# microsoft/GenerativeImage2Text

Hardware: AMD Instinct MI355X
Metric: captions/sec whole-node (GIT_BASE 224px bs=64/GPU greedy len=20) (higher is better)
Workload: dtype f16; 1 GPU; GIT_BASE 224px bs=64/GPU greedy max_len=20 frames=1; global_batch=64, parallelism=dp1, decode_steps_per_caption=19, seq_len_returned=20, hip_graph=True, contexts_in_flight=4, layernorm_folded=True, library=libgitmi_f16.so, encoder_chains=2, schedule=mixed

## Files before the change

generativeimage2text_amd/csrc/abi_ops.hip:

```cpp
#include "../../include/gitmi.h"
#include "abi_common.h"
#include "gitmi_common.h"
#include "launchers.h"

#include <hip/hip_runtime.h>

using namespace gitmi;

#ifdef GITMI_EXPERIMENT
#include "../../include/gitmi_experiment.h"
#define GITMI_EXP_EXPORT extern "C"
#else
#define GITMI_EXP_EXPORT [[maybe_unused]] static
#endif

static inline int round_up(int x, int m) { return (x + m - 1) / m * m; }

extern "C" int gitmi_operand_dtype(void);
static const char* dtype_name(int dtype) {
    return dtype == GITMI_DTYPE_F32 ? "fp32" : dtype == GITMI_DTYPE_BF16 ? "bf16" : dtype == GITMI_DTYPE_F16 ? "fp16" : "unknown";
}
static int check_dtype(const char* op, const char* arg, int dtype) {
    if (dtype == GITMI_DTYPE_F32 || dtype == gitmi_operand_dtype()) return 0;
    return fail("%s: %s is %s (%d), but this library's 16-bit operands are %s (libgitmi%s.so)", op, arg, dtype_name(dtype), dtype,
// ... 47 lines not shown
extern "C" int gitmi_op_layernorm(const float* x, const float* gamma, const float* beta, float eps, void* y_t,
                                  float* y_f32, int rows, int D, int out_dtype, void* stream) {
    if (y_t) RCK(check_dtype("op_layernorm", "out_dtype", out_dtype));
    HIPCK(launch_layernorm(x, D, gamma, beta, eps, nullptr, y_t, D, out_dtype == GITMI_DTYPE_F32, y_f32, D, rows, D, 0, 0,
                           0, (hipStream_t)stream));
    return 0;
}
extern "C" int gitmi_op_attention(const void* qkv, void* out, int B, int N, int H, int dtype, int impl, void* stream) {
    RCK(check_dtype("op_attention", "dtype", dtype));
    const size_t esz = dtype == GITMI_DTYPE_F32 ? 4 : 2;
    const int D = H * 64;
    AttnFullArgs a{};
    a.q = qkv;
    a.k = (const char*)qkv + (size_t)D * esz;
    a.v = (const char*)qkv + (size_t)2 * D * esz;
    a.out = out;
    a.ldq = a.ldk = a.ldv = 3 * D;
    a.ldo = D;
    a.N = N; a.H = H; a.scale = 0.125f;
    if (attn_decode_configure() != hipSuccess) return fail("configure failed");
    HIPCK(launch_attn_full(a, B, dtype == GITMI_DTYPE_F32, impl, (hipStream_t)stream));
    return 0;
}

#ifdef GITMI_EXPERIMENT
static int g_dgemm_dbg = 0;
GITMI_EXP_EXPORT int gitmi_debug_set_dgemm(int dbg) { g_dgemm_dbg = dbg; return 0; }
#else
static const int g_dgemm_dbg = 0;
#endif
extern "C" int gitmi_op_dgemm(const void* A, const void* W, const float* bias, const float* colsum, const float* stats,
                              int strips, float eps, void* C, int c_frag, int M, int N, int K, int act, int strips_per_wg,
                              void* stream) {
    DGemmArgs g{};
    g.dbg = g_dgemm_dbg;
    g.strips_per_wg = strips_per_wg;
    g.c_frag = c_frag;
    if (c_frag && N % 32) return fail("op_dgemm: a fragment-major output needs N %% 32 == 0");
    g.A = (const unsigned short*)A; g.lda = K; g.W = (const unsigned short*)W; g.bias = bias;
    if (stats) { g.colsum = colsum; g.stats_in = (const float2*)stats; g.strips_in = strips; g.inv_d = 1.0f / (float)K; g.eps_in = eps; }
    g.C = C; g.ldc = N; g.act = act; g.M = M; g.N = N; g.K = K;
    if (K % 32) return fail("op_dgemm: K must be a multiple of 32");
    HIPCK(launch_dgemm(g, (hipStream_t)stream));
    return 0;
}
extern "C" int gitmi_op_dgemm_res(const void* A, const void* W, const float* bias, const float* res_x, const float* res_stats,
// ... 302 lines not shown
```

generativeimage2text_amd/csrc/kernels_attn.hip:

```cpp
#include "gitmi_common.h"
#include "launchers.h"
#include <type_traits>

namespace gitmi {

constexpr int HD = 64;

template <typename T>
__global__ __launch_bounds__(256) void attn_full_valu_kernel(AttnFullArgs a) {
    __shared__ float Ks[64][HD + 1];
    __shared__ float Vs[64][HD + 1];
    __shared__ float qs[16][HD];
    __shared__ float ps[16][64];

    const int tid = threadIdx.x, lane = tid & 63, wave = tid >> 6;
    const int h = blockIdx.y, b = blockIdx.z;
    const int q0 = blockIdx.x * 16;
    const T* Q = reinterpret_cast<const T*>(a.q);
    const T* K = reinterpret_cast<const T*>(a.k);
    const T* V = reinterpret_cast<const T*>(a.v);
    T* O = reinterpret_cast<T*>(a.out);
    const size_t base_row = (size_t)b * a.N;
    const int n = a.ntok ? a.ntok[b] : a.N;
    if (q0 >= n) {
// ... 179 lines not shown
                    o_acc[t][dt] = mfma16(vf.v, pf, o_acc[t][dt]);
                }
            }
        }
    }

#pragma unroll
    for (int t = 0; t < QT; ++t) {
        const int qr = qbase + (t * 4 + wave) * 16 + l15;
        if (qr < a.N) {
            const float inv = qr < n ? 1.0f / l_run[t] : 0.f;
            bf16_t* op = O + (base_row + qr) * a.ldo + h * HD;
#pragma unroll
            for (int dt = 0; dt < 4; ++dt) {
                uint2 tt;
                tt.x = pack2bf(o_acc[t][dt][0] * inv, o_acc[t][dt][1] * inv);
                tt.y = pack2bf(o_acc[t][dt][2] * inv, o_acc[t][dt][3] * inv);
                *reinterpret_cast<uint2*>(op + dt * 16 + lg * 4) = tt;
            }
        }
    }
}

template <int NSUB, bool RAGGED = false>
__global__ __launch_bounds__(256, 2) void attn_full_mfma_short_kernel(AttnFullArgs a) {
    constexpr int NK = NSUB * 16;
    constexpr int NB = (NSUB + 1) / 2;
    constexpr int LDV = NB * 32 + 8;
    static_assert((LDV / 8) % 2 == 1, "V^T row stride must be an odd multiple of 16 bytes");
    __shared__ __attribute__((aligned(16))) bf16_t Ks[NK * FA_LDK];
    __shared__ __attribute__((aligned(16))) bf16_t Vt[HD * LDV];

    const int tid = threadIdx.x, lane = tid & 63, wave = tid >> 6;
    const int l15 = lane & 15, lg = lane >> 4;
    const int h = blockIdx.x, b = blockIdx.y;
    const bf16_t* Q = reinterpret_cast<const bf16_t*>(a.q);
    const bf16_t* K = reinterpret_cast<const bf16_t*>(a.k);
    const bf16_t* V = reinterpret_cast<const bf16_t*>(a.v);
    bf16_t* O = reinterpret_cast<bf16_t*>(a.out);
    const size_t base_row = (size_t)b * a.N;
    const int n = RAGGED ? a.ntok[b] : a.N;
    if constexpr (RAGGED) {
        for (int i = tid; i < (a.N - n) * 8; i += 256) {
            const int qr = n + (i >> 3);
            *reinterpret_cast<u32x4_t*>(O + (base_row + qr) * a.ldo + h * HD + (i & 7) * 8) = u32x4_t{0u, 0u, 0u, 0u};
        }
    }

#pragma unroll
    for (int it = 0; it < (NK * 8 + 255) / 256; ++it) {
        int idx = tid + it * 256;
        const bool ok = idx < NK * 8;
        idx = ok ? idx : NK * 8 - 1;
        const int key = idx >> 3, c = idx & 7;
        const int kr = key < n ? key : n - 1;
        const u32x4_t kc = *reinterpret_cast<const u32x4_t*>(K + (base_row + kr) * a.ldk + h * HD + c * 8);
        if (ok) *reinterpret_cast<u32x4_t*>(Ks + key * FA_LDK + c * 8) = kc;
    }
#pragma unroll
    for (int it = 0; it < (NB * 8 * 8 + 255) / 256; ++it) {
        int task = tid + it * 256;
        const bool ok = task < NB * 8 * 8;
        task = ok ? task : NB * 8 * 8 - 1;
        const int kg = task % (NB * 8), c = task / (NB * 8);
        u32x4_t vc[4];
#pragma unroll
        for (int e = 0; e < 4; ++e) {
            const int key = kg * 4 + e;
            const int kr = key < n ? key : n - 1;
            vc[e] = *reinterpret_cast<const u32x4_t*>(V + (base_row + kr) * a.ldv + h * HD + c * 8);
            if (key >= n) vc[e] = u32x4_t{0u, 0u, 0u, 0u};
        }
        if (ok) {
#pragma unroll
            for (int w = 0; w < 4; ++w) {
                uint2 even, odd;
                even.x = (vc[0][w] & 0xffffu) | (vc[1][w] << 16);
                even.y = (vc[2][w] & 0xffffu) | (vc[3][w] << 16);
                odd.x = (vc[0][w] >> 16) | (vc[1][w] & 0xffff0000u);
                odd.y = (vc[2][w] >> 16) | (vc[3][w] & 0xffff0000u);
                *reinterpret_cast<uint2*>(Vt + (c * 8 + 2 * w) * LDV + kg * 4) = even;
                *reinterpret_cast<uint2*>(Vt + (c * 8 + 2 * w + 1) * LDV + kg * 4) = odd;
            }
        }
    }
    __syncthreads();

    const int nqt = (n + 15) >> 4;
    const float c2 = a.scale * 1.4426950408889634f;

    auto process = [&](auto nt_c, int t0) {
        constexpr int NT = decltype(nt_c)::value;
        bf16x8_t qf[NT][2];
#pragma unroll
        for (int u = 0; u < NT; ++u) {
            int qr = (t0 + 4 * u) * 16 + l15;
            qr = qr < n ? qr : n - 1;
            const bf16_t* qp = Q + (base_row + qr) * a.ldq + h * HD + lg * 8;
            qf[u][0] = *reinterpret_cast<const bf16x8_t*>(qp);
            qf[u][1] = *reinterpret_cast<const bf16x8_t*>(qp + 32);
        }
        f32x4_t sacc[NT][NSUB];
#pragma unroll
        for (int st_ = 0; st_ < NSUB; ++st_) {
            const bf16x8_t kf0 = *reinterpret_cast<const bf16x8_t*>(Ks + (st_ * 16 + l15) * FA_LDK + lg * 8);
            const bf16x8_t kf1 = *reinterpret_cast<const bf16x8_t*>(Ks + (st_ * 16 + l15) * FA_LDK + 32 + lg * 8);
#pragma unroll
            for (int u = 0; u < NT; ++u) {
                sacc[u][st_] = mfma16(kf0, qf[u][0], f32x4_t{0.f, 0.f, 0.f, 0.f});
                sacc[u][st_] = mfma16(kf1, qf[u][1], sacc[u][st_]);
            }
            if constexpr (NSUB > 13) { if (st_ % 4 == 3) __builtin_amdgcn_sched_barrier(0); }
        }
        float inv_l[NT];
#pragma unroll
        for (int u = 0; u < NT; ++u) {
            if constexpr (RAGGED) {
#pragma unroll
                for (int st_ = 0; st_ < NSUB; ++st_)
#pragma unroll
                    for (int r = 0; r < 4; ++r)
                        if (st_ * 16 + lg * 4 + r >= n) sacc[u][st_][r] = -INFINITY;
            } else {
#pragma unroll
                for (int r = 0; r < 4; ++r)
                    if ((NSUB - 1) * 16 + lg * 4 + r >= a.N) sacc[u][NSUB - 1][r] = -INFINITY;
            }
            float m = -INFINITY;
#pragma unroll
            for (int st_ = 0; st_ < NSUB; ++st_)
#pragma unroll
                for (int r = 0; r < 4; ++r) m = fmaxf(m, sacc[u][st_][r]);
            m = fmaxf(m, __shfl_xor(m, 16, 64));
            m = fmaxf(m, __shfl_xor(m, 32, 64));
            const float mc = m * c2;
            float psum = 0.f;
#pragma unroll
            for (int st_ = 0; st_ < NSUB; ++st_)
#pragma unroll
                for (int r = 0; r < 4; ++r) {
                    const float p = __builtin_amdgcn_exp2f(sacc[u][st_][r] * c2 - mc);
                    sacc[u][st_][r] = p;
                    psum += p;
                }
            psum += __shfl_xor(psum, 16, 64);
            psum += __shfl_xor(psum, 32, 64);
            inv_l[u] = 1.0f / psum;
        }
        uint32_t pk2[NT][NSUB][2];
#pragma unroll
        for (int u = 0; u < NT; ++u)
#pragma unroll
            for (int st_ = 0; st_ < NSUB; ++st_) {
                pk2[u][st_][0] = pack2bf(sacc[u][st_][0], sacc[u][st_][1]);
                pk2[u][st_][1] = pack2bf(sacc[u][st_][2], sacc[u][st_][3]);
            }
        f32x4_t o_acc[NT][4];
#pragma unroll
        for (int u = 0; u < NT; ++u)
#pragma unroll
            for (int dt = 0; dt < 4; ++dt) o_acc[u][dt] = f32x4_t{0.f, 0.f, 0.f, 0.f};
#pragma unroll
        for (int blk = 0; blk < NB; ++blk) {
            bf16x8_t pf[NT];
#pragma unroll
            for (int u = 0; u < NT; ++u) {
                union { bf16x8_t v; uint32_t w[4]; } pk;
                pk.w[0] = pk2[u][2 * blk][0];
                pk.w[1] = pk2[u][2 * blk][1];
                const bool has1 = 2 * blk + 1 < NSUB;
                const int s1 = has1 ? 2 * blk + 1 : 0;
                pk.w[2] = has1 ? pk2[u][s1][0] : 0u;
                pk.w[3] = has1 ? pk2[u][s1][1] : 0u;
                pf[u] = pk.v;
            }
#pragma unroll
            for (int dt = 0; dt < 4; ++dt) {
                union { bf16x8_t v; uint2 h2[2]; } vf;
                const bf16_t* vp = Vt + (dt * 16 + l15) * LDV + blk * 32 + lg * 4;
                vf.h2[0] = *reinterpret_cast<const uint2*>(vp);
                vf.h2[1] = *reinterpret_cast<const uint2*>(vp + 16);
#pragma unroll
                for (int u = 0; u < NT; ++u)
                    o_acc[u][dt] = mfma16(vf.v, pf[u], o_acc[u][dt]);
            }
        }
#pragma unroll
        for (int u = 0; u < NT; ++u) {
            const int qr = (t0 + 4 * u) * 16 + l15;
            if (qr < n) {
                bf16_t* op = O + (base_row + qr) * a.ldo + h * HD;
#pragma unroll
                for (int dt = 0; dt < 4; ++dt) {
                    uint2 tt;
                    tt.x = pack2bf(o_acc[u][dt][0] * inv_l[u], o_acc[u][dt][1] * inv_l[u]);
                    tt.y = pack2bf(o_acc[u][dt][2] * inv_l[u], o_acc[u][dt][3] * inv_l[u]);
                    *reinterpret_cast<uint2*>(op + dt * 16 + lg * 4) = tt;
                }
            }
        }
    };

    for (int t0 = wave; t0 < nqt; t0 += 8) {
        if (t0 + 4 < nqt) process(std::integral_constant<int, 2>{}, t0);
        else process(std::integral_constant<int, 1>{}, t0);
    }
}

template <typename T>
__global__ void kv_repack_kernel(const T* __restrict__ qkv, T* __restrict__ kh, T* __restrict__ vh, int B, int N, int H,
                                 int d) {
    constexpr int CH = 16 / (int)sizeof(T);
    constexpr int CPH = HD / CH;
    const size_t per = (size_t)B * H * N * CPH;
    for (size_t i = blockIdx.x * (size_t)blockDim.x + threadIdx.x; i < 2 * per; i += (size_t)gridDim.x * blockDim.x) {
        const int kv = i >= per;
        size_t r = kv ? i - per : i;
        const int c = (int)(r % CPH); r /= CPH;
        const int n = (int)(r % N); r /= N;
        const int h = (int)(r % H);
        const int b = (int)(r / H);
        const T* src = qkv + ((size_t)b * N + n) * 3 * d + (kv ? 2 : 1) * d + h * HD + c * CH;
        T* dst = (kv ? vh : kh) + (((size_t)b * H + h) * N + n) * HD + c * CH;
        *reinterpret_cast<u32x4_t*>(dst) = *reinterpret_cast<const u32x4_t*>(src);
    }
}

template <typename T> struct Raw8;
// ... 231 lines not shown
        }
    }
    __syncthreads();
    for (int i = tid; i < k * HD; i += 256) {
        const int j = i / HD, dd = i % HD;
        float mm = -INFINITY;
#pragma unroll
        for (int w = 0; w < 4; ++w) mm = fmaxf(mm, part[w][j][HD]);
        float num = 0.f, den = 0.f;
#pragma unroll
        for (int w = 0; w < 4; ++w) {
            const float mw = part[w][j][HD];
            const float aw = mw == -INFINITY ? 0.f : fast_exp(mw - mm);
            num += aw * part[w][j][dd];
            den += aw * part[w][j][HD + 1];
        }
        if constexpr (sizeof(T) == 2) {
            if (a.out_frag) { O[frag_offset(row0 + j, h * HD + dd, a.d >> 5)] = f2bf(num / den); continue; }
        }
        st<T>(O + (size_t)(row0 + j) * a.d + h * HD + dd, num / den);
    }
}

hipError_t launch_attn_full(const AttnFullArgs& a, int B, bool is_f32, int impl, hipStream_t s) {
    if (B <= 0 || a.N <= 0) return hipSuccess;
    if (impl == 1) {
        if (is_f32) return hipErrorInvalidValue;
        const int nsub = (a.N + 15) / 16;
        if (nsub == 13 && a.ntok) hipLaunchKernelGGL((attn_full_mfma_short_kernel<13, true>), dim3(a.H, B), dim3(256), 0, s, a);
        else if (nsub == 13) hipLaunchKernelGGL(attn_full_mfma_short_kernel<13>, dim3(a.H, B), dim3(256), 0, s, a);
        else if (nsub == 17 && a.ntok) hipLaunchKernelGGL((attn_full_mfma_short_kernel<17, true>), dim3(a.H, B), dim3(256), 0, s, a);
        else if (nsub == 17) hipLaunchKernelGGL(attn_full_mfma_short_kernel<17>, dim3(a.H, B), dim3(256), 0, s, a);
        else hipLaunchKernelGGL(attn_full_mfma_kernel, dim3((a.N + 255) / 256, a.H, B), dim3(256), 0, s, a);
    } else if (impl == 2) {
        if (is_f32) return hipErrorInvalidValue;
        hipLaunchKernelGGL(attn_full_mfma_kernel, dim3((a.N + 255) / 256, a.H, B), dim3(256), 0, s, a);
    } else if (is_f32) {
        hipLaunchKernelGGL(attn_full_valu_kernel<float>, dim3((a.N + 15) / 16, a.H, B), dim3(256), 0, s, a);
    } else {
        hipLaunchKernelGGL(attn_full_valu_kernel<bf16_t>, dim3((a.N + 15) / 16, a.H, B), dim3(256), 0, s, a);
    }
    return hipGetLastError();
}

hipError_t launch_kv_repack(const void* qkv, void* kh, void* vh, int B, int N, int H, int d, bool is_f32, hipStream_t s) {
    if (B <= 0 || N <= 0) return hipSuccess;
    const size_t total = 2 * (size_t)B * H * N * (is_f32 ? 16 : 8);
    size_t grid = (total + 255) / 256;
    grid = grid > 8192 ? 8192 : grid;
    if (is_f32) hipLaunchKernelGGL(kv_repack_kernel<float>, dim3((int)grid), dim3(256), 0, s, (const float*)qkv, (float*)kh,
                                   (float*)vh, B, N, H, d);
    else hipLaunchKernelGGL(kv_repack_kernel<bf16_t>, dim3((int)grid), dim3(256), 0, s, (const bf16_t*)qkv, (bf16_t*)kh,
                            (bf16_t*)vh, B, N, H, d);
    return hipGetLastError();
}

hipError_t attn_decode_configure() { return hipSuccess; }

size_t attn_decode_lds_bytes(int beams, int N_img, int pos) {
// ... 22 lines not shown
```

generativeimage2text_amd/csrc/launchers.h:

```cpp
#pragma once
#include <hip/hip_runtime.h>
#include <stddef.h>

namespace gitmi {

struct GemmArgs {
    const void* A; const void* W; const float* bias; const float* res; void* C;
    int M, N, K;
    int lda, ldc, ldr;
    int act;
    int tiles_n, nwg;
    int ng;
    int dbg;
    int out_f16;
    int shared;
    const float2* ln_part; int ln_nparts; const float* ln_colsum; float ln_inv_d, ln_eps;
    float2* part_out;
    const float2* res_part; int res_nparts; const float* res_gamma; const float* res_beta; float res_inv_d, res_eps;
};
bool gemm_uses_p8(const GemmArgs& g, bool in_f32, bool out_f32);
hipError_t launch_gemm(const GemmArgs& g, bool in_f32, bool out_f32, hipStream_t s);
hipError_t launch_gemm_p8(GemmArgs g, bool out_f32, hipStream_t s);
bool gemm_p8_supports(const GemmArgs& g);
int gemm_p8_cost(const GemmArgs& g, int bm);
// ... 54 lines not shown
                                  int nparts, hipStream_t s);
hipError_t launch_layernorm_s16(const void* x, int ldx, const float* gamma, const float* beta, float eps,
                                const float* add_after, void* y_t, int ld_t, bool t_is_f32, void* y_s, int ld_s,
                                int rows, int D, int map_n_in, int map_n_out, int map_off, hipStream_t s);
hipError_t launch_embed_ln(const int* ids, int ld_ids, int pos, const float* words, const float* positions,
                           const float* gamma, const float* beta, float eps, float* h_f, void* h_t, bool t_is_f32,
                           int R, int D, int vocab, bool frag, hipStream_t s);
hipError_t launch_frag_pack(const void* src_bf16, void* dst_bf16, int rows, int rows_out, int K, hipStream_t s);
hipError_t launch_convert_pad(const float* src, void* dst, bool dst_f32, size_t rows, int K, int Kpad,
                              hipStream_t s);
hipError_t launch_convert(const void* src, bool src_f32, void* dst, bool dst_f32, size_t n, hipStream_t s);
hipError_t launch_chain_input(const float* x, void* xb_frag, float2* stats, int R, int d, hipStream_t s);
hipError_t launch_copy_f32(const float* src, int lds, float* dst, int ldd, int rows, int cols, hipStream_t s);
hipError_t launch_fill_i32(int* dst, int value, int n, hipStream_t s);

struct AttnFullArgs {
    const void* q; const void* k; const void* v; void* out;
    int ldq, ldk, ldv, ldo;
    int N, H;
    float scale;
    const int* ntok;
};
hipError_t launch_attn_full(const AttnFullArgs& a, int B, bool is_f32, int impl, hipStream_t s);

struct AttnDecodeArgs {
    const void* qkv; const void* img_k; const void* img_v; void* txt_k; void* txt_v; void* out;
    const int* kv_src;
    const int* img_of;
    int ld_src;
    int d;
    int N_img, T_max, pos, beams;
    int N_pad;
    int out_frag;
    float scale;
    int dbg;
    int pairs_per_wg;
    int pairs_per_wave;
    int stream_wgs;
    int n_pairs;
    int waves_per_pair;
    const int* ntok;
};
hipError_t launch_kv_repack(const void* qkv, void* kh, void* vh, int B, int N, int H, int d, bool is_f32, hipStream_t s);
size_t attn_decode_lds_bytes(int beams, int N_img, int pos);
hipError_t launch_attn_decode(const AttnDecodeArgs& a, int B, int H, bool is_f32, hipStream_t s);
hipError_t launch_kv_repack_frag(const void* qkv, void* kf, void* vt, int B, int N, int N_pad, int H, int d, hipStream_t s);
// ... 92 lines not shown
```

generativeimage2text_amd/engine.py:

```python
from __future__ import annotations

import ctypes as C
import os
from typing import Dict, List, Mapping, Optional, Sequence, Tuple

import torch

_HERE = os.path.dirname(os.path.abspath(__file__))
LIB_PATH = os.path.join(_HERE, "libgitmi.so")
LIB_PATH_F16 = os.path.join(_HERE, "libgitmi_f16.so")
LIB_PATH_EXP = os.path.join(_HERE, "libgitmi_exp.so")

PREC_BF16, PREC_F32 = 0, 1
DTYPE_F32, DTYPE_BF16, DTYPE_F16 = 0, 1, 2
DTYPE_F16_STREAM = 3
SEARCH_AUTOREGRESSIVE, SEARCH_GENERATOR, SEARCH_TRIE = 0, 1, 2
SEARCH_SCORE = 3
SEARCH_ATTEND = 4
ACT_NONE, ACT_QUICKGELU, ACT_GELU_ERF = 0, 1, 2

EXPORTED_SYMBOLS = [
    "gitmi_abi_version", "gitmi_last_error", "gitmi_create", "gitmi_destroy", "gitmi_load_tensor",
    "gitmi_finalize_weights", "gitmi_encode_frames", "gitmi_prefill", "gitmi_step_logits",
    "gitmi_generate", "gitmi_search_begin", "gitmi_search_rows", "gitmi_search_advance",
    "gitmi_search_finish", "gitmi_profile_enable", "gitmi_profile_read", "gitmi_set_graph",
    "gitmi_op_gemm", "gitmi_op_layernorm", "gitmi_op_attention", "gitmi_op_dgemm", "gitmi_op_dgemm_res",
    "gitmi_op_vocab_topm", "gitmi_clone", "gitmi_op_attn_decode", "gitmi_preprocess_image",
    "gitmi_set_image_shape", "gitmi_preprocess_image_to", "gitmi_generate_prefixed", "gitmi_set_temporal_embedding", "gitmi_op_kv_repack", "gitmi_set_encode_after", "gitmi_op_sample_rows",
    "gitmi_search_done_count", "gitmi_set_trie", "gitmi_operand_dtype", "gitmi_set_shared_device", "gitmi_preprocess_batch",
    "gitmi_set_ln_fold", "gitmi_op_gemm_ln",
]
EXPERIMENT_SYMBOLS = [
    "gitmi_debug_import_stage", "gitmi_debug_head_from", "gitmi_debug_set_gemm_impl", "gitmi_debug_set_dgemm",
    "gitmi_debug_score_attn", "gitmi_debug_score_head", "gitmi_debug_attention_ragged", "gitmi_debug_attn_decode_ragged",
    "gitmi_debug_vocab_topm_rules", "gitmi_debug_search_begin_prefixed", "gitmi_debug_search_advance_lists", "gitmi_debug_read_hidden",
    "gitmi_debug_im2col", "gitmi_debug_pos_resize", "gitmi_debug_vit_assemble", "gitmi_debug_ragged_front", "gitmi_debug_zero_pad_rows",
    "gitmi_debug_layernorm_map", "gitmi_debug_score_attn_map",
]


class GitmiConfig(C.Structure):
    _fields_ = [(n, C.c_int32) for n in (
        "image_size", "patch", "vit_width", "vit_layers", "vit_heads", "dec_hidden", "dec_layers",
        "dec_heads", "dec_ffn", "vocab", "max_pos", "num_frames", "sos", "eos", "precision",
        "max_batch", "max_beams", "max_frames", "max_text_len", "max_image_pixels", "max_image_tokens")]


class GitmiSearch(C.Structure):
    _fields_ = [("kind", C.c_int32), ("beam_size", C.c_int32), ("per_node_beam_size", C.c_int32),
                ("max_steps", C.c_int32), ("length_penalty", C.c_double),
                ("do_sample", C.c_int32), ("top_k", C.c_int32), ("top_p", C.c_double), ("temperature", C.c_double),
                ("seed", C.c_uint64), ("repetition_penalty", C.c_double),
                ("num_keep_best", C.c_int32), ("reserved_", C.c_int32)]


class GitmiProfile(C.Structure):
    _fields_ = [("vit_ms", C.c_float), ("prefill_ms", C.c_float), ("decode_ms", C.c_float),
                ("total_ms", C.c_float), ("gemm_ms", C.c_float), ("gemm_launches", C.c_int32),
                ("gemm_flops", C.c_double), ("vit_gemm_ms", C.c_float), ("vit_gemm_launches", C.c_int32),
                ("vit_gemm_flops", C.c_double), ("decode_step_ms", C.c_float), ("decode_steps", C.c_int32),
# ... 803 lines not shown
    _ck(_experiment_only(lib, "gitmi_debug_vocab_topm_rules")(
        *ops, eps, *shape, _ptr(ids), 0 if ids is None else int(ids.shape[1]), int(cur_len), _ptr(plen), int(beams),
        int(suppress_kind), float(rep_penalty), *outs, int(max_wgs), _stream()), lib)
    return result


def set_gemm_impl(impl: int) -> None:
    lib = load_library()
    _ck(_experiment_only(lib, "gitmi_debug_set_gemm_impl")(int(impl)), lib)


def op_attn_decode(qkv, img_k, img_v, txt_k, txt_v, kv_src, B, H, N_img, T_max, pos, beams, dbg=0):
    lib = _op_library(qkv.dtype, img_k.dtype, img_v.dtype, txt_k.dtype, txt_v.dtype, fp32_ok=True)
    R, d = B * beams, H * 64
    out = torch.empty(R, d, device=qkv.device, dtype=qkv.dtype)
    if qkv.dtype != torch.float32 and img_k.dim() == 4:
        img_k, img_v = kv_repack(img_k, img_v)
    _ck(lib.gitmi_op_attn_decode(qkv.data_ptr(), img_k.data_ptr(), img_v.data_ptr(), txt_k.data_ptr(), txt_v.data_ptr(),
                                 kv_src.data_ptr(), out.data_ptr(), B, H, N_img, T_max, pos, beams, _torch_dtype_code(qkv),
                                 dbg, _stream()), lib)
    return out


def op_attention_ragged(qkv: torch.Tensor, ntok, B: int, N: int, H: int, impl: int) -> torch.Tensor:
    lib = load_library()
    nt = torch.as_tensor(ntok, dtype=torch.int32).to(qkv.device)
    out = torch.empty(B * N, H * 64, device=qkv.device, dtype=qkv.dtype)
    _ck(_experiment_only(lib, "gitmi_debug_attention_ragged")(qkv.data_ptr(), out.data_ptr(), nt.data_ptr(), B, N, H,
                                                              _torch_dtype_code(qkv), impl, _stream()), lib)
    return out


def op_attn_decode_ragged(qkv, img_k, img_v, txt_k, txt_v, kv_src, ntok, B, H, N_img, T_max, pos, beams):
    lib = load_library()
    R, d = B * beams, H * 64
    nt = torch.as_tensor(ntok, dtype=torch.int32).to(qkv.device)
    out = torch.empty(R, d, device=qkv.device, dtype=qkv.dtype)
    if qkv.dtype != torch.float32 and img_k.dim() == 4:
        img_k, img_v = kv_repack(img_k, img_v)
    _ck(_experiment_only(lib, "gitmi_debug_attn_decode_ragged")(qkv.data_ptr(), img_k.data_ptr(), img_v.data_ptr(), txt_k.data_ptr(),
                                                                txt_v.data_ptr(), kv_src.data_ptr(), out.data_ptr(), nt.data_ptr(), B,
                                                                H, N_img, T_max, pos, beams, _torch_dtype_code(qkv), _stream()), lib)
    return out


def op_score_attn(qkv: torch.Tensor, img_kv: torch.Tensor, image_of: torch.Tensor, Q: int, H: int, N_img: int,
# ... 144 lines not shown
```

include/gitmi_experiment.h:

```cpp
#ifndef GITMI_EXPERIMENT_H_
#define GITMI_EXPERIMENT_H_
#include "gitmi.h"
#ifdef __cplusplus
extern "C" {
#endif

int  gitmi_debug_import_stage(gitmi_engine* dst, gitmi_engine* src, int stage, void* stream);
int  gitmi_debug_head_from(gitmi_engine* dst, gitmi_engine* src, int R, float* logits_out, void* stream);

int  gitmi_debug_set_gemm_impl(int impl);

int  gitmi_debug_set_dgemm(int dbg);

int  gitmi_debug_score_attn(const void* qkv, const void* img_kv, const int* image_of, void* out, int Q, int H, int N_img, int Lp,
                            int dtype, void* stream);
int  gitmi_debug_score_attn_map(const void* qkv, const void* img_kv, const int* image_of, const int* ntok, float* out, int Q, int H,
                                int N_img, int Lp, int dtype, void* stream);
int  gitmi_debug_score_head(const void* A, const void* W, const float* bias, const int* tgt, int M, int V, int K, int dtype,
                            float* out, void* stream);

int  gitmi_debug_attention_ragged(const void* qkv, void* out, const int* ntok, int B, int N, int H, int dtype, int impl, void* stream);
int  gitmi_debug_attn_decode_ragged(const void* qkv, const void* img_k, const void* img_v, void* txt_k, void* txt_v,
                                    const int* kv_src, void* out, const int* ntok, int B, int H, int N_img, int T_max, int pos,
                                    int beams, int dtype, void* stream);

int  gitmi_debug_vocab_topm_rules(const void* A, const void* W, const float* bias, const float* colsum, const float* stats,
                                  int strips, float eps, int M, int V, int K, int cols_per_wg, int mtop, const int* ids, int ld_ids,
                                  int cur_len, const int* plen, int beams, int suppress_kind, float rep_penalty, float* part_val,
                                  int* part_idx, float* part_lse, float* logits_out, int max_wgs, void* stream);
int  gitmi_debug_search_begin_prefixed(gitmi_engine* e, const gitmi_search* sp, int B, const int64_t* start_host, int ld,
                                       const int32_t* plen_host, int vocab, void* stream);
int  gitmi_debug_search_advance_lists(gitmi_engine* e, const float* part_val, const int* part_idx, const float* part_lse,
                                      int nparts, int slots, int embed, void* stream);
int  gitmi_debug_read_hidden(gitmi_engine* e, int R, float* hf_out, void* ht_out, int* ht_frag, int* ht_dtype, void* stream);

// ... 18 lines not shown
```

Measured before the change: 11620 captions/s.

## Add persistent double-buffered short attention kernel overlapping next head's K/V load

For the non-ragged short-sequence encoder attention (13 or 17 key subtiles), impl 1 now launches a persistent 512-thread kernel with one workgroup per CU. Each workgroup loops over (batch, head) pairs and prefetches the next pair's K/V into registers while computing the current one, then writes them into a second LDS buffer. The tile math is factored into shared helpers, and the old per-pair kernel moves to experimental impl 3. The aim is to hide global-load latency and cut workgroup launch overhead. The cost is doubled LDS, more register pressure and one workgroup per CU, which can limit occupancy.

```diff
diff --git a/generativeimage2text_amd/csrc/abi_ops.hip b/generativeimage2text_amd/csrc/abi_ops.hip
--- a/generativeimage2text_amd/csrc/abi_ops.hip
+++ b/generativeimage2text_amd/csrc/abi_ops.hip
@@ -93,6 +93,8 @@
     HIPCK(launch_attn_full(a, B, dtype == GITMI_DTYPE_F32, impl, (hipStream_t)stream));
     return 0;
 }
+
+GITMI_EXP_EXPORT int gitmi_debug_attn_short_grid(int pairs) { return attn_full_short_grid(pairs); }
 
 #ifdef GITMI_EXPERIMENT
 static int g_dgemm_dbg = 0;
diff --git a/generativeimage2text_amd/csrc/kernels_attn.hip b/generativeimage2text_amd/csrc/kernels_attn.hip
--- a/generativeimage2text_amd/csrc/kernels_attn.hip
+++ b/generativeimage2text_amd/csrc/kernels_attn.hip
@@ -225,188 +225,310 @@
     }
 }
 
+template <int NSUB> struct ShortGeom {
+    static constexpr int NK = NSUB * 16;
+    static constexpr int NB = (NSUB + 1) / 2;
+    static constexpr int LDV = NB * 32 + 8;
+    static_assert((LDV / 8) % 2 == 1, "V^T row stride must be an odd multiple of 16 bytes");
+    static constexpr int KS = NK * FA_LDK;
+    static constexpr int VT = HD * LDV;
+};
+
+struct ShortPair {
+    int h, n;
+    size_t base_row;
+};
+template <bool RAGGED> __device__ __forceinline__ ShortPair short_pair(const AttnFullArgs& a, int b, int h) {
+    ShortPair p;
+    p.h = h;
+    p.n = RAGGED ? a.ntok[b] : a.N;
+    p.base_row = (size_t)b * a.N;
+    return p;
+}
+
+template <int NSUB, int NTHR> struct ShortStage {
+    using G = ShortGeom<NSUB>;
+    static constexpr int KCH = G::NK * 8, VTASK = G::NB * 8 * 8;
+    static constexpr int KIT = KCH / NTHR, KREM = KCH - KIT * NTHR;
+    static constexpr int VIT = VTASK / NTHR, VREM = VTASK - VIT * NTHR;
+    static_assert(VREM % 64 == 0 && KREM % 4 == 0 && VREM + KREM / 4 <= NTHR, "the shared last block does not fit");
+    u32x4_t kc[KIT];
+    u32x4_t vc[VIT + 1][4];
+
+    static __device__ __forceinline__ u32x4_t chunk(const bf16_t* M, int ld, const ShortPair& p, int key, int c) {
+        const int kr = key < p.n ? key : p.n - 1;
+        return *reinterpret_cast<const u32x4_t*>(M + (p.base_row + kr) * ld + p.h * HD + c * 8);
+    }
+    __device__ __forceinline__ void load(const AttnFullArgs& a, const ShortPair& p, int tid) {
+        const bf16_t* K = reinterpret_cast<const bf16_t*>(a.k);
+        const bf16_t* V = reinterpret_cast<const bf16_t*>(a.v);
+#pragma unroll
+        for (int it = 0; it < KIT; ++it) {
+            const int idx = tid + it * NTHR;
+            kc[it] = chunk(K, a.ldk, p, idx >> 3, idx & 7);
+        }
+#pragma unroll
+        for (int it = 0; it <= VIT; ++it) {
+            const int task = tid + it * NTHR;
+            if (it < VIT || tid < VREM) {
+                const int kg = task % (G::NB * 8), c = task / (G::NB * 8);
+#pragma unroll
+                for (int e = 0; e < 4; ++e) vc[it][e] = chunk(V, a.ldv, p, kg * 4 + e, c);
+            } else if (tid - VREM < KREM / 4) {
+                const int idx = KIT * NTHR + (tid - VREM) * 4;
+#pragma unroll
+                for (int e = 0; e < 4; ++e) vc[it][e] = chunk(K, a.ldk, p, idx >> 3, (idx & 7) + e);
+            }
+        }
+    }
+    __device__ __forceinline__ void store(bf16_t* Ks, bf16_t* Vt, int tid, int n) const {
+#pragma unroll
+        for (int it = 0; it < KIT; ++it) {
+            const int idx = tid + it * NTHR;
+            *reinterpret_cast<u32x4_t*>(Ks + (idx >> 3) * FA_LDK + (idx & 7) * 8) = kc[it];
+        }
+#pragma unroll
+        for (int it = 0; it <= VIT; ++it) {
+            const int task = tid + it * NTHR;
+            if (it < VIT || tid < VREM) {
+                const int kg = task % (G::NB * 8), c = task / (G::NB * 8);
+                u32x4_t v[4];
+#pragma unroll
+                for (int e = 0; e < 4; ++e) v[e] = kg * 4 + e < n ? vc[it][e] : u32x4_t{0u, 0u, 0u, 0u};
+#pragma unroll
+                for (int w = 0; w < 4; ++w) {
+                    uint2 even, odd;
+                    even.x = (v[0][w] & 0xffffu) | (v[1][w] << 16);
+                    even.y = (v[2][w] & 0xffffu) | (v[3][w] << 16);
+                    odd.x = (v[0][w] >> 16) | (v[1][w] & 0xffff0000u);
+                    odd.y = (v[2][w] >> 16) | (v[3][w] & 0xffff0000u);
+                    *reinterpret_cast<uint2*>(Vt + (c * 8 + 2 * w) * G::LDV + kg * 4) = even;
+                    *reinterpret_cast<uint2*>(Vt + (c * 8 + 2 * w + 1) * G::LDV + kg * 4) = odd;
+                }
+            } else if (tid - VREM < KREM / 4) {
+                const int idx = KIT * NTHR + (tid - VREM) * 4;
+#pragma unroll
+                for (int e = 0; e < 4; ++e)
+                    *reinterpret_cast<u32x4_t*>(Ks + (idx >> 3) * FA_LDK + ((idx & 7) + e) * 8) = vc[it][e];
+            }
+        }
+    }
+};
+
+template <int NT>
+__device__ __forceinline__ void short_load_q(const AttnFullArgs& a, const ShortPair& p, int t0, int ts, int l15, int lg,
+                                             bf16x8_t (&qf)[NT][2]) {
+    const bf16_t* Q = reinterpret_cast<const bf16_t*>(a.q);
+#pragma unroll
+    for (int u = 0; u < NT; ++u) {
+        int qr = (t0 + ts * u) * 16 + l15;
+        qr = qr < p.n ? qr : p.n - 1;
+        const bf16_t* qp = Q + (p.base_row + qr) * a.ldq + p.h * HD + lg * 8;
+        qf[u][0] = *reinterpret_cast<const bf16x8_t*>(qp);
+        qf[u][1] = *reinterpret_cast<const bf16x8_t*>(qp + 32);
+    }
+}
+
+template <int NSUB, bool RAGGED, int NT, int QS>
+__device__ __forceinline__ void short_tile_math(const AttnFullArgs& a, const ShortPair& p, const bf16_t* Ks, const bf16_t* Vt,
+                                                const bf16x8_t (&qf)[QS][2], int t0, int ts, int l15, int lg) {
+    using G = ShortGeom<NSUB>;
+    constexpr int NB = G::NB, LDV = G::LDV;
+    bf16_t* O = reinterpret_cast<bf16_t*>(a.out);
+    const int n = p.n;
+    const float c2 = a.scale * 1.4426950408889634f;
+    f32x4_t sacc[NT][NSUB];
+#pragma unroll
+    for (int st_ = 0; st_ < NSUB; ++st_) {
+        const bf16x8_t kf0 = *reinterpret_cast<const bf16x8_t*>(Ks + (st_ * 16 + l15) * FA_LDK + lg * 8);
+        const bf16x8_t kf1 = *reinterpret_cast<const bf16x8_t*>(Ks + (st_ * 16 + l15) * FA_LDK + 32 + lg * 8);
+#pragma unroll
+        for (int u = 0; u < NT; ++u) {
+            sacc[u][st_] = mfma16(kf0, qf[u][0], f32x4_t{0.f, 0.f, 0.f, 0.f});
+            sacc[u][st_] = mfma16(kf1, qf[u][1], sacc[u][st_]);
+        }
+        if constexpr (NSUB > 13) { if (st_ % 4 == 3) __builtin_amdgcn_sched_barrier(0); }
+    }
+    float inv_l[NT];
+#pragma unroll
+    for (int u = 0; u < NT; ++u) {
+        if constexpr (RAGGED) {
+#pragma unroll
+            for (int st_ = 0; st_ < NSUB; ++st_)
+#pragma unroll
+                for (int r = 0; r < 4; ++r)
+                    if (st_ * 16 + lg * 4 + r >= n) sacc[u][st_][r] = -INFINITY;
+        } else {
+#pragma unroll
+            for (int r = 0; r < 4; ++r)
+                if ((NSUB - 1) * 16 + lg * 4 + r >= a.N) sacc[u][NSUB - 1][r] = -INFINITY;
+        }
+        float m = -INFINITY;
+#pragma unroll
+        for (int st_ = 0; st_ < NSUB; ++st_)
+#pragma unroll
+            for (int r = 0; r < 4; ++r) m = fmaxf(m, sacc[u][st_][r]);
+        m = fmaxf(m, __shfl_xor(m, 16, 64));
+        m = fmaxf(m, __shfl_xor(m, 32, 64));
+        const float mc = m * c2;
+        float psum = 0.f;
+#pragma unroll
+        for (int st_ = 0; st_ < NSUB; ++st_)
+#pragma unroll
+            for (int r = 0; r < 4; ++r) {
+                const float pr = __builtin_amdgcn_exp2f(sacc[u][st_][r] * c2 - mc);
+                sacc[u][st_][r] = pr;
+                psum += pr;
+            }
+        psum += __shfl_xor(psum, 16, 64);
+        psum += __shfl_xor(psum, 32, 64);
+        inv_l[u] = 1.0f / psum;
+    }
+    uint32_t pk2[NT][NSUB][2];
+#pragma unroll
+    for (int u = 0; u < NT; ++u)
+#pragma unroll
+        for (int st_ = 0; st_ < NSUB; ++st_) {
+            pk2[u][st_][0] = pack2bf(sacc[u][st_][0], sacc[u][st_][1]);
+            pk2[u][st_][1] = pack2bf(sacc[u][st_][2], sacc[u][st_][3]);
+        }
+    f32x4_t o_acc[NT][4];
+#pragma unroll
+    for (int u = 0; u < NT; ++u)
+#pragma unroll
+        for (int dt = 0; dt < 4; ++dt) o_acc[u][dt] = f32x4_t{0.f, 0.f, 0.f, 0.f};
+#pragma unroll
+    for (int blk = 0; blk < NB; ++blk) {
+        bf16x8_t pf[NT];
+#pragma unroll
+        for (int u = 0; u < NT; ++u) {
+            union { bf16x8_t v; uint32_t w[4]; } pk;
+            pk.w[0] = pk2[u][2 * blk][0];
+            pk.w[1] = pk2[u][2 * blk][1];
+            const bool has1 = 2 * blk + 1 < NSUB;
+            const int s1 = has1 ? 2 * blk + 1 : 0;
+            pk.w[2] = has1 ? pk2[u][s1][0] : 0u;
+            pk.w[3] = has1 ? pk2[u][s1][1] : 0u;
+            pf[u] = pk.v;
+        }
+#pragma unroll
+        for (int dt = 0; dt < 4; ++dt) {
+            union { bf16x8_t v; uint2 h2[2]; } vf;
+            const bf16_t* vp = Vt + (dt * 16 + l15) * LDV + blk * 32 + lg * 4;
+            vf.h2[0] = *reinterpret_cast<const uint2*>(vp);
+            vf.h2[1] = *reinterpret_cast<const uint2*>(vp + 16);
+#pragma unroll
+            for (int u = 0; u < NT; ++u)
+                o_acc[u][dt] = mfma16(vf.v, pf[u], o_acc[u][dt]);
+        }
+    }
+#pragma unroll
+    for (int u = 0; u < NT; ++u) {
+        const int qr = (t0 + ts * u) * 16 + l15;
+        if (qr < n) {
+            bf16_t* op = O + (p.base_row + qr) * a.ldo + p.h * HD;
+#pragma unroll
+            for (int dt = 0; dt < 4; ++dt) {
+                uint2 tt;
+                tt.x = pack2bf(o_acc[u][dt][0] * inv_l[u], o_acc[u][dt][1] * inv_l[u]);
+                tt.y = pack2bf(o_acc[u][dt][2] * inv_l[u], o_acc[u][dt][3] * inv_l[u]);
+                *reinterpret_cast<uint2*>(op + dt * 16 + lg * 4) = tt;
+            }
+        }
+    }
+}
+
+template <int NTHR> __device__ __forceinline__ void short_zero_pad(const AttnFullArgs& a, const ShortPair& p, int tid) {
+    bf16_t* O = reinterpret_cast<bf16_t*>(a.out);
+    for (int i = tid; i < (a.N - p.n) * 8; i += NTHR) {
+        const int qr = p.n + (i >> 3);
+        *reinterpret_cast<u32x4_t*>(O + (p.base_row + qr) * a.ldo + p.h * HD + (i & 7) * 8) = u32x4_t{0u, 0u, 0u, 0u};
+    }
+}
+
+#define SHORT_LDS_BARRIER()                                \
+    do {                                                   \
+        asm volatile("s_waitcnt lgkmcnt(0)" ::: "memory"); \
+        __builtin_amdgcn_s_barrier();                      \
+    } while (0)
+
+template <int NSUB>
+__global__ __launch_bounds__(512) void attn_full_mfma_short_persistent_kernel(AttnFullArgs a, int pairs) {
+    using G = ShortGeom<NSUB>;
+    constexpr bool RAGGED = false;
+    constexpr int TS = 8;
+    constexpr int NTM = NSUB <= 13 ? 2 : 1;
+    __shared__ __attribute__((aligned(16))) bf16_t Ks[2 * G::KS];
+    __shared__ __attribute__((aligned(16))) bf16_t Vt[2 * G::VT];
+
+    const int tid = threadIdx.x, lane = tid & 63, wave = tid >> 6;
+    const int l15 = lane & 15, lg = lane >> 4;
+    const int grid = gridDim.x;
+
+    int pair = blockIdx.x;
+    ShortPair p = short_pair<RAGGED>(a, pair / a.H, pair % a.H);
+    ShortStage<NSUB, 512> stg;
+    bf16x8_t qf[NTM][2];
+    stg.load(a, p, tid);
+    short_load_q<NTM>(a, p, wave, TS, l15, lg, qf);
+    stg.store(Ks, Vt, tid, p.n);
+    SHORT_LDS_BARRIER();
+
+    int cur = 0;
+    for (;;) {
+        const int next = pair + grid;
+        const bool has_next = next < pairs;
+        ShortPair pn = p;
+        if (has_next) {
+            pn = short_pair<RAGGED>(a, next / a.H, next % a.H);
+            stg.load(a, pn, tid);
+        }
+        __builtin_amdgcn_sched_barrier(0);
+
+        const bf16_t* ks = Ks + cur * G::KS;
+        const bf16_t* vt = Vt + cur * G::VT;
+        const int nqt = (p.n + 15) >> 4;
+        if (NTM == 2 && wave + TS < nqt) short_tile_math<NSUB, RAGGED, NTM>(a, p, ks, vt, qf, wave, TS, l15, lg);
+        else if (wave < nqt) short_tile_math<NSUB, RAGGED, 1>(a, p, ks, vt, qf, wave, TS, l15, lg);
+        for (int t0 = wave + NTM * TS; t0 < nqt; t0 += NTM * TS) {
+            bf16x8_t qx[NTM][2];
+            short_load_q<NTM>(a, p, t0, TS, l15, lg, qx);
+            if (NTM == 2 && t0 + TS < nqt) short_tile_math<NSUB, RAGGED, NTM>(a, p, ks, vt, qx, t0, TS, l15, lg);
+            else short_tile_math<NSUB, RAGGED, 1>(a, p, ks, vt, qx, t0, TS, l15, lg);
+        }
+        if (!has_next) break;
+
+        __builtin_amdgcn_sched_barrier(0);
+        stg.store(Ks + (cur ^ 1) * G::KS, Vt + (cur ^ 1) * G::VT, tid, pn.n);
+        short_load_q<NTM>(a, pn, wave, TS, l15, lg, qf);
+        SHORT_LDS_BARRIER();
+        pair = next;
+        p = pn;
+        cur ^= 1;
+    }
+}
+
 template <int NSUB, bool RAGGED = false>
 __global__ __launch_bounds__(256, 2) void attn_full_mfma_short_kernel(AttnFullArgs a) {
-    constexpr int NK = NSUB * 16;
-    constexpr int NB = (NSUB + 1) / 2;
-    constexpr int LDV = NB * 32 + 8;
-    static_assert((LDV / 8) % 2 == 1, "V^T row stride must be an odd multiple of 16 bytes");
-    __shared__ __attribute__((aligned(16))) bf16_t Ks[NK * FA_LDK];
-    __shared__ __attribute__((aligned(16))) bf16_t Vt[HD * LDV];
+    using G = ShortGeom<NSUB>;
+    __shared__ __attribute__((aligned(16))) bf16_t Ks[G::KS];
+    __shared__ __attribute__((aligned(16))) bf16_t Vt[G::VT];
 
     const int tid = threadIdx.x, lane = tid & 63, wave = tid >> 6;
     const int l15 = lane & 15, lg = lane >> 4;
-    const int h = blockIdx.x, b = blockIdx.y;
-    const bf16_t* Q = reinterpret_cast<const bf16_t*>(a.q);
-    const bf16_t* K = reinterpret_cast<const bf16_t*>(a.k);
-    const bf16_t* V = reinterpret_cast<const bf16_t*>(a.v);
-    bf16_t* O = reinterpret_cast<bf16_t*>(a.out);
-    const size_t base_row = (size_t)b * a.N;
-    const int n = RAGGED ? a.ntok[b] : a.N;
-    if constexpr (RAGGED) {
-        for (int i = tid; i < (a.N - n) * 8; i += 256) {
-            const int qr = n + (i >> 3);
-            *reinterpret_cast<u32x4_t*>(O + (base_row + qr) * a.ldo + h * HD + (i & 7) * 8) = u32x4_t{0u, 0u, 0u, 0u};
-        }
-    }
-
-#pragma unroll
-    for (int it = 0; it < (NK * 8 + 255) / 256; ++it) {
-        int idx = tid + it * 256;
-        const bool ok = idx < NK * 8;
-        idx = ok ? idx : NK * 8 - 1;
-        const int key = idx >> 3, c = idx & 7;
-        const int kr = key < n ? key : n - 1;
-        const u32x4_t kc = *reinterpret_cast<const u32x4_t*>(K + (base_row + kr) * a.ldk + h * HD + c * 8);
-        if (ok) *reinterpret_cast<u32x4_t*>(Ks + key * FA_LDK + c * 8) = kc;
-    }
-#pragma unroll
-    for (int it = 0; it < (NB * 8 * 8 + 255) / 256; ++it) {
-        int task = tid + it * 256;
-        const bool ok = task < NB * 8 * 8;
-        task = ok ? task : NB * 8 * 8 - 1;
-        const int kg = task % (NB * 8), c = task / (NB * 8);
-        u32x4_t vc[4];
-#pragma unroll
-        for (int e = 0; e < 4; ++e) {
-            const int key = kg * 4 + e;
-            const int kr = key < n ? key : n - 1;
-            vc[e] = *reinterpret_cast<const u32x4_t*>(V + (base_row + kr) * a.ldv + h * HD + c * 8);
-            if (key >= n) vc[e] = u32x4_t{0u, 0u, 0u, 0u};
-        }
-        if (ok) {
-#pragma unroll
-            for (int w = 0; w < 4; ++w) {
-                uint2 even, odd;
-                even.x = (vc[0][w] & 0xffffu) | (vc[1][w] << 16);
-                even.y = (vc[2][w] & 0xffffu) | (vc[3][w] << 16);
-                odd.x = (vc[0][w] >> 16) | (vc[1][w] & 0xffff0000u);
-                odd.y = (vc[2][w] >> 16) | (vc[3][w] & 0xffff0000u);
-                *reinterpret_cast<uint2*>(Vt + (c * 8 + 2 * w) * LDV + kg * 4) = even;
-                *reinterpret_cast<uint2*>(Vt + (c * 8 + 2 * w + 1) * LDV + kg * 4) = odd;
-            }
-        }
-    }
+    const ShortPair p = short_pair<RAGGED>(a, blockIdx.y, blockIdx.x);
+    if constexpr (RAGGED) short_zero_pad<256>(a, p, tid);
+    ShortStage<NSUB, 256> stg;
+    stg.load(a, p, tid);
+    stg.store(Ks, Vt, tid, p.n);
     __syncthreads();
 
-    const int nqt = (n + 15) >> 4;
-    const float c2 = a.scale * 1.4426950408889634f;
-
-    auto process = [&](auto nt_c, int t0) {
-        constexpr int NT = decltype(nt_c)::value;
-        bf16x8_t qf[NT][2];
-#pragma unroll
-        for (int u = 0; u < NT; ++u) {
-            int qr = (t0 + 4 * u) * 16 + l15;
-            qr = qr < n ? qr : n - 1;
-            const bf16_t* qp = Q + (base_row + qr) * a.ldq + h * HD + lg * 8;
-            qf[u][0] = *reinterpret_cast<const bf16x8_t*>(qp);
-            qf[u][1] = *reinterpret_cast<const bf16x8_t*>(qp + 32);
-        }
-        f32x4_t sacc[NT][NSUB];
-#pragma unroll
-        for (int st_ = 0; st_ < NSUB; ++st_) {
-            const bf16x8_t kf0 = *reinterpret_cast<const bf16x8_t*>(Ks + (st_ * 16 + l15) * FA_LDK + lg * 8);
-            const bf16x8_t kf1 = *reinterpret_cast<const bf16x8_t*>(Ks + (st_ * 16 + l15) * FA_LDK + 32 + lg * 8);
-#pragma unroll
-            for (int u = 0; u < NT; ++u) {
-                sacc[u][st_] = mfma16(kf0, qf[u][0], f32x4_t{0.f, 0.f, 0.f, 0.f});
-                sacc[u][st_] = mfma16(kf1, qf[u][1], sacc[u][st_]);
-            }
-            if constexpr (NSUB > 13) { if (st_ % 4 == 3) __builtin_amdgcn_sched_barrier(0); }
-        }
-        float inv_l[NT];
-#pragma unroll
-        for (int u = 0; u < NT; ++u) {
-            if constexpr (RAGGED) {
-#pragma unroll
-                for (int st_ = 0; st_ < NSUB; ++st_)
-#pragma unroll
-                    for (int r = 0; r < 4; ++r)
-                        if (st_ * 16 + lg * 4 + r >= n) sacc[u][st_][r] = -INFINITY;
-            } else {
-#pragma unroll
-                for (int r = 0; r < 4; ++r)
-                    if ((NSUB - 1) * 16 + lg * 4 + r >= a.N) sacc[u][NSUB - 1][r] = -INFINITY;
-            }
-            float m = -INFINITY;
-#pragma unroll
-            for (int st_ = 0; st_ < NSUB; ++st_)
-#pragma unroll
-                for (int r = 0; r < 4; ++r) m = fmaxf(m, sacc[u][st_][r]);
-            m = fmaxf(m, __shfl_xor(m, 16, 64));
-            m = fmaxf(m, __shfl_xor(m, 32, 64));
-            const float mc = m * c2;
-            float psum = 0.f;
-#pragma unroll
-            for (int st_ = 0; st_ < NSUB; ++st_)
-#pragma unroll
-                for (int r = 0; r < 4; ++r) {
-                    const float p = __builtin_amdgcn_exp2f(sacc[u][st_][r] * c2 - mc);
-                    sacc[u][st_][r] = p;
-                    psum += p;
-                }
-            psum += __shfl_xor(psum, 16, 64);
-            psum += __shfl_xor(psum, 32, 64);
-            inv_l[u] = 1.0f / psum;
-        }
-        uint32_t pk2[NT][NSUB][2];
-#pragma unroll
-        for (int u = 0; u < NT; ++u)
-#pragma unroll
-            for (int st_ = 0; st_ < NSUB; ++st_) {
-                pk2[u][st_][0] = pack2bf(sacc[u][st_][0], sacc[u][st_][1]);
-                pk2[u][st_][1] = pack2bf(sacc[u][st_][2], sacc[u][st_][3]);
-            }
-        f32x4_t o_acc[NT][4];
-#pragma unroll
-        for (int u = 0; u < NT; ++u)
-#pragma unroll
-            for (int dt = 0; dt < 4; ++dt) o_acc[u][dt] = f32x4_t{0.f, 0.f, 0.f, 0.f};
-#pragma unroll
-        for (int blk = 0; blk < NB; ++blk) {
-            bf16x8_t pf[NT];
-#pragma unroll
-            for (int u = 0; u < NT; ++u) {
-                union { bf16x8_t v; uint32_t w[4]; } pk;
-                pk.w[0] = pk2[u][2 * blk][0];
-                pk.w[1] = pk2[u][2 * blk][1];
-                const bool has1 = 2 * blk + 1 < NSUB;
-                const int s1 = has1 ? 2 * blk + 1 : 0;
-                pk.w[2] = has1 ? pk2[u][s1][0] : 0u;
-                pk.w[3] = has1 ? pk2[u][s1][1] : 0u;
-                pf[u] = pk.v;
-            }
-#pragma unroll
-            for (int dt = 0; dt < 4; ++dt) {
-                union { bf16x8_t v; uint2 h2[2]; } vf;
-                const bf16_t* vp = Vt + (dt * 16 + l15) * LDV + blk * 32 + lg * 4;
-                vf.h2[0] = *reinterpret_cast<const uint2*>(vp);
-                vf.h2[1] = *reinterpret_cast<const uint2*>(vp + 16);
-#pragma unroll
-                for (int u = 0; u < NT; ++u)
-                    o_acc[u][dt] = mfma16(vf.v, pf[u], o_acc[u][dt]);
-            }
-        }
-#pragma unroll
-        for (int u = 0; u < NT; ++u) {
-            const int qr = (t0 + 4 * u) * 16 + l15;
-            if (qr < n) {
-                bf16_t* op = O + (base_row + qr) * a.ldo + h * HD;
-#pragma unroll
-                for (int dt = 0; dt < 4; ++dt) {
-                    uint2 tt;
-                    tt.x = pack2bf(o_acc[u][dt][0] * inv_l[u], o_acc[u][dt][1] * inv_l[u]);
-                    tt.y = pack2bf(o_acc[u][dt][2] * inv_l[u], o_acc[u][dt][3] * inv_l[u]);
-                    *reinterpret_cast<uint2*>(op + dt * 16 + lg * 4) = tt;
-                }
-            }
-        }
-    };
-
+    const int nqt = (p.n + 15) >> 4;
     for (int t0 = wave; t0 < nqt; t0 += 8) {
-        if (t0 + 4 < nqt) process(std::integral_constant<int, 2>{}, t0);
-        else process(std::integral_constant<int, 1>{}, t0);
+        bf16x8_t qf[2][2];
+        short_load_q<2>(a, p, t0, 4, l15, lg, qf);
+        if (t0 + 4 < nqt) short_tile_math<NSUB, RAGGED, 2>(a, p, Ks, Vt, qf, t0, 4, l15, lg);
+        else short_tile_math<NSUB, RAGGED, 1>(a, p, Ks, Vt, qf, t0, 4, l15, lg);
     }
 }
 
@@ -684,9 +806,42 @@
     }
 }
 
+int attn_full_short_grid(int pairs) {
+    static int cus[64];
+    int dev = 0;
+    if (hipGetDevice(&dev) != hipSuccess || dev < 0 || dev >= 64) return 0;
+    int n = __atomic_load_n(&cus[dev], __ATOMIC_RELAXED);
+    if (n <= 0) {
+        if (hipDeviceGetAttribute(&n, hipDeviceAttributeMultiprocessorCount, dev) != hipSuccess || n <= 0) return 0;
+        __atomic_store_n(&cus[dev], n, __ATOMIC_RELAXED);
+    }
+    return pairs < n ? pairs : n;
+}
+
+template <int NSUB>
+static hipError_t launch_short_persistent(const AttnFullArgs& a, int B, hipStream_t s) {
+    const int pairs = B * a.H;
+    const int grid = attn_full_short_grid(pairs);
+    if (grid <= 0) return hipErrorInvalidDevice;
+    hipLaunchKernelGGL(attn_full_mfma_short_persistent_kernel<NSUB>, dim3(grid), dim3(512), 0, s, a, pairs);
+    return hipGetLastError();
+}
+
 hipError_t launch_attn_full(const AttnFullArgs& a, int B, bool is_f32, int impl, hipStream_t s) {
     if (B <= 0 || a.N <= 0) return hipSuccess;
     if (impl == 1) {
+        if (is_f32) return hipErrorInvalidValue;
+        const int nsub = (a.N + 15) / 16;
+        if (nsub == 13 && a.ntok) hipLaunchKernelGGL((attn_full_mfma_short_kernel<13, true>), dim3(a.H, B), dim3(256), 0, s, a);
+        else if (nsub == 13) return launch_short_persistent<13>(a, B, s);
+        else if (nsub == 17 && a.ntok) hipLaunchKernelGGL((attn_full_mfma_short_kernel<17, true>), dim3(a.H, B), dim3(256), 0, s, a);
+        else if (nsub == 17) return launch_short_persistent<17>(a, B, s);
+        else hipLaunchKernelGGL(attn_full_mfma_kernel, dim3((a.N + 255) / 256, a.H, B), dim3(256), 0, s, a);
+    } else if (impl == 2) {
+        if (is_f32) return hipErrorInvalidValue;
+        hipLaunchKernelGGL(attn_full_mfma_kernel, dim3((a.N + 255) / 256, a.H, B), dim3(256), 0, s, a);
+    } else if (impl == 3) {
+#ifdef GITMI_EXPERIMENT
         if (is_f32) return hipErrorInvalidValue;
         const int nsub = (a.N + 15) / 16;
         if (nsub == 13 && a.ntok) hipLaunchKernelGGL((attn_full_mfma_short_kernel<13, true>), dim3(a.H, B), dim3(256), 0, s, a);
@@ -694,9 +849,9 @@
         else if (nsub == 17 && a.ntok) hipLaunchKernelGGL((attn_full_mfma_short_kernel<17, true>), dim3(a.H, B), dim3(256), 0, s, a);
         else if (nsub == 17) hipLaunchKernelGGL(attn_full_mfma_short_kernel<17>, dim3(a.H, B), dim3(256), 0, s, a);
         else hipLaunchKernelGGL(attn_full_mfma_kernel, dim3((a.N + 255) / 256, a.H, B), dim3(256), 0, s, a);
-    } else if (impl == 2) {
-        if (is_f32) return hipErrorInvalidValue;
-        hipLaunchKernelGGL(attn_full_mfma_kernel, dim3((a.N + 255) / 256, a.H, B), dim3(256), 0, s, a);
+#else
+        return hipErrorInvalidValue;
+#endif
     } else if (is_f32) {
         hipLaunchKernelGGL(attn_full_valu_kernel<float>, dim3((a.N + 15) / 16, a.H, B), dim3(256), 0, s, a);
     } else {
diff --git a/generativeimage2text_amd/csrc/launchers.h b/generativeimage2text_amd/csrc/launchers.h
--- a/generativeimage2text_amd/csrc/launchers.h
+++ b/generativeimage2text_amd/csrc/launchers.h
@@ -100,6 +100,7 @@
     const int* ntok;
 };
 hipError_t launch_attn_full(const AttnFullArgs& a, int B, bool is_f32, int impl, hipStream_t s);
+int attn_full_short_grid(int pairs);
 
 struct AttnDecodeArgs {
     const void* qkv; const void* img_k; const void* img_v; void* txt_k; void* txt_v; void* out;
diff --git a/generativeimage2text_amd/engine.py b/generativeimage2text_amd/engine.py
--- a/generativeimage2text_amd/engine.py
+++ b/generativeimage2text_amd/engine.py
@@ -35,7 +35,7 @@
     "gitmi_debug_score_attn", "gitmi_debug_score_head", "gitmi_debug_attention_ragged", "gitmi_debug_attn_decode_ragged",
     "gitmi_debug_vocab_topm_rules", "gitmi_debug_search_begin_prefixed", "gitmi_debug_search_advance_lists", "gitmi_debug_read_hidden",
     "gitmi_debug_im2col", "gitmi_debug_pos_resize", "gitmi_debug_vit_assemble", "gitmi_debug_ragged_front", "gitmi_debug_zero_pad_rows",
-    "gitmi_debug_layernorm_map", "gitmi_debug_score_attn_map",
+    "gitmi_debug_layernorm_map", "gitmi_debug_score_attn_map", "gitmi_debug_attn_short_grid",
 ]
 
 
@@ -885,6 +885,10 @@
     return out
 
 
+def attn_short_grid(pairs: int) -> int:
+    return int(_experiment_only(load_library(), "gitmi_debug_attn_short_grid")(int(pairs)))
+
+
 def op_attention_ragged(qkv: torch.Tensor, ntok, B: int, N: int, H: int, impl: int) -> torch.Tensor:
     lib = load_library()
     nt = torch.as_tensor(ntok, dtype=torch.int32).to(qkv.device)
diff --git a/include/gitmi_experiment.h b/include/gitmi_experiment.h
--- a/include/gitmi_experiment.h
+++ b/include/gitmi_experiment.h
@@ -11,6 +11,8 @@
 int  gitmi_debug_set_gemm_impl(int impl);
 
 int  gitmi_debug_set_dgemm(int dbg);
+
+int  gitmi_debug_attn_short_grid(int pairs);
 
 int  gitmi_debug_score_attn(const void* qkv, const void* img_kv, const int* image_of, void* out, int Q, int H, int N_img, int Lp,
                             int dtype, void* stream);
```

Result: slower. 11450 captions/s (-1.4%).
